# google/lyra

Measured on AMD Instinct MI355X. Metric: 20ms 16kHz frames/sec encode+decode (whole node) at batch 4096; xRT/stream, higher is better.
Workload: dtype f32+i8 (fp32 and int8 layers exactly as the reference graphs)

## Files before the change

lyra_amd/csrc/dec_stages.h:

```cpp
#ifndef LYRA_AMD_CSRC_DEC_STAGES_H_
#define LYRA_AMD_CSRC_DEC_STAGES_H_
#include "resblock_q.h"

namespace lyra {

namespace {
constexpr int SD0 = 8;
constexpr int FS = 72;
constexpr int CS2 = 264;
constexpr int QS = 288;
constexpr int QS5 = 544;
constexpr int NTD0 = 512;
constexpr int MTD0 = (2 * SD0) / 16;
constexpr int FB_FLOATS = 3 * 16 * FS;
constexpr int XF_FLOATS = 2 * SD0 * CS2;
constexpr int H8_BYTES = 16 * QS5;
constexpr int QB_BYTES = 2 * SD0 * QS;
constexpr int QA_BYTES = 2 * 16 * QS;
constexpr int NLR = 6, NADD = 2;
static_assert(SD0 == 8, "tile size the index math below supports");
}

__host__ __device__ constexpr size_t dec_s0_lds() {
  return (size_t)(FB_FLOATS + XF_FLOATS) * 4 + H8_BYTES + 3 * QB_BYTES + QA_BYTES + 2 * SD0 * 4 + NLR * 256 +
// ... 358 lines not shown
      }
    }
  }
}

__host__ __device__ constexpr size_t dec_s1_lds() { return (size_t)(4 * SD1 * CS1 + 4 * SD1 * CS1 + 4 * SD1 * CS1 + 5 * SD1 * 72) * 4 + 2 * SD1 * 4; }

__device__ __forceinline__ void dec_s1_body(const DecS1P& P, const float* __restrict__ in0,
                                            const int32_t* __restrict__ ids, int B, uint8_t* __restrict__ state,
                                            float* __restrict__ out1, int code_bytes, int tile = (int)blockIdx.x) {
  extern __shared__ __attribute__((aligned(16))) float smem[];
  float* XB = smem;
  float* DB = XB + 4 * SD1 * CS1;
  float* PB = DB + 4 * SD1 * CS1;
  float* SB = PB + 4 * SD1 * CS1;
  int* sids = reinterpret_cast<int*>(SB + 5 * SD1 * 72);
  int* sphase = sids + SD1;
  const int tid = threadIdx.x, wave = tid >> 6;
  const int b0 = tile * SD1;
  LYRA_TSTAMP(50);
  int my_id = 0;
  if (tid < SD1) my_id = ids[min(b0 + tid, B - 1)];
  constexpr int XIN = (4 * SD1 * 32) / NTD1;
  static_assert((4 * SD1 * 32) % NTD1 == 0 && (4 * SD1 * 32) / NTD1 >= 1, "the unrolled input prefetch covers the stage input only when the thread count divides it");
  f32x4 xin[XIN];
#pragma unroll
  for (int k = 0; k < XIN; ++k) {
    const int idx = tid + k * NTD1;
    int p4 = idx & 31, s = (idx >> 5) & (SD1 - 1), t = (idx >> 5) / SD1;
    int sb = min(s, B - 1 - b0);
    xin[k] = *goff<const f32x4>(in0 + (size_t)b0 * 512, (uint32_t)(((sb * 4 + t) * 128 + p4 * 4) * 4));
  }
  if (tid < SD1) {
    sids[tid] = my_id;
    sphase[tid] = *reinterpret_cast<const int*>(state + (size_t)max(my_id, 0) * st::D1_BYTES + st::PHASE);
  }
  const auto warm = l2_warm<NTD1, 2>(P.warm);
  const auto warm_code = code_warm<NTD1>(code_bytes);
#pragma unroll
  for (int k = 0; k < XIN; ++k) {
    const int idx = tid + k * NTD1;
    int p4 = idx & 31, s = (idx >> 5) & (SD1 - 1), t = (idx >> 5) / SD1;
    *reinterpret_cast<f32x4*>(&XB[(t * SD1 + s) * CS1 + p4 * 4]) = xin[k];
  }
  LYRA_SYNC_KEEP();
  TileCtx cx{state, sids, sphase, B - b0, st::D1_BYTES};
  const auto H0 = hist128_prefetch<SD1, NTD1>(cx, 1, st::D_R1_0);
  for (int idx = tid; idx < 5 * SD1 * 16; idx += NTD1) {
    int p4 = idx & 15, s = (idx >> 4) & (SD1 - 1), j = (idx >> 4) / SD1;
    *reinterpret_cast<f32x4*>(&SB[(j * SD1 + s) * 72 + p4 * 4]) =
        *cx.at<const f32x4>(cx.soff(s) + (uint32_t)(st::D_UP2 + (j * 64 + p4 * 4) * 4));
  }
  __syncthreads();
  LYRA_TSTAMP(51);
  LYRA_WSTAMP(111);
  resblocks128<SD1, NTD1>(XB, DB, PB, cx, P.dw, P.pw, P.cv, st::D_R1_0, st::D_R1_1, st::D_R1_2, H0);
  LYRA_TSTAMP(52);
  LYRA_WSTAMP(112);
  for (int idx = tid; idx < 4 * SD1 * 32; idx += NTD1) {
    int p4 = idx & 31, rs = idx >> 5;
    f32x4* x = reinterpret_cast<f32x4*>(&XB[rs * CS1 + p4 * 4]);
    *x = lrelu4(*x);
  }
  __syncthreads();
  LYRA_TSTAMP(53);
  LYRA_WSTAMP(113);
  constexpr int HEAD_TILES = NTD1 == 256 ? 5 : 3;
  static_assert((NTD1 / 64) * HEAD_TILES * 256 <= 2 * 4 * SD1 * CS1, "head scratch fits into DB + PB");
  float* HB = DB + wave * (HEAD_TILES * 4 * 64);
  if (NTD1 == 256) dec_s1_tconv<5>(XB, SB, P, cx, b0, out1, wave * 5, HB);
  else if (wave < 4) dec_s1_tconv<3>(XB, SB, P, cx, b0, out1, wave * 3, HB);
  else dec_s1_tconv<2>(XB, SB, P, cx, b0, out1, 12 + (wave - 4) * 2, HB);
  if (tid < SD1 && cx.valid(tid)) {
    int ph = sphase[tid] + 1;
    *cx.at<int>(cx.soff(tid) + (uint32_t)(st::PHASE)) = ph >= st::PHASE_MOD ? 0 : ph;
  }
  l2_warm_sink(warm, state, B);
  l2_warm_sink(warm_code, state, B);
}

namespace {
constexpr int CS0 = 72;
}
__host__ __device__ constexpr size_t dec_s2_lds(int sd2) { return (size_t)(27 * sd2 * CS0 + sd2 * 48) * 4 + 64; }

template <int SD2>
__device__ __forceinline__ void dec_s2_body(const DecS2P& P, const float* __restrict__ in1,
                                            const int32_t* __restrict__ ids, int B, uint8_t* __restrict__ state,
                                            int16_t* __restrict__ pcm, int code_bytes, int tile = (int)blockIdx.x) {
  constexpr int NTD2 = 64 * SD2;
  extern __shared__ __attribute__((aligned(16))) float smem[];
  float* XB = smem;
  float* SB = XB + 27 * SD2 * CS0;
  int* sids = reinterpret_cast<int*>(SB + SD2 * 48);
  const int tid = threadIdx.x, lane = tid & 63, wave = tid >> 6;
  const int m = lane & 15, q = lane >> 4;
  const int b0 = tile * SD2;
  LYRA_TSTAMP(60);
  int my_id = 0;
  if (tid < SD2) my_id = ids[min(b0 + tid, B - 1)];
  const int wn = wave & 3, wm = wave >> 2;
  [[maybe_unused]] const int ncol = wn * 16 + (lane & 15);
  f32x4 xr[5][1];
#pragma unroll
  for (int i = 0; i < 5; ++i) {
    const int R = (wm * 5 + i) * 16 + m, t = R / SD2, s = R & (SD2 - 1);
    const int sb = min(s, B - 1 - b0);
    xr[i][0] = *goff<const f32x4>(in1 + (size_t)b0 * 1280, (uint32_t)(((sb * 20 + t) * 64 + wn * 16 + q * 4) * 4));
  }
  if (tid < SD2) sids[tid] = my_id;
  const auto warm = l2_warm<NTD2, 1>(P.warm);
  const auto warm_code = code_warm<NTD2>(code_bytes);
  LYRA_SYNC_KEEP();
  TileCtx cx{state, sids, nullptr, B - b0, st::D2_BYTES};
  for (int idx = tid; idx < 7 * SD2 * 16; idx += NTD2) {
    int p4 = idx & 15, s = (idx >> 4) & (SD2 - 1), j = (idx >> 4) / SD2;
    int row = j < 3 ? j : 20 + j;
    *reinterpret_cast<f32x4*>(&XB[(row * SD2 + s) * CS0 + p4 * 4]) = (f32x4){0.f, 0.f, 0.f, 0.f};
  }
  for (int idx = tid; idx < SD2 * 48; idx += NTD2) {
    int s = idx / 48, i = idx - s * 48;
    SB[idx] = *cx.at<const float>(cx.soff(s) + (uint32_t)(st::D_UP3 + i * 4));
  }
  LYRA_TSTAMP(61);
  resblocks64r<SD2, NTD2>(xr, XB + 3 * SD2 * CS0, cx, P.dw, P.pw, P.cv, st::D_R2_0, st::D_R2_1, st::D_R2_2);
  LYRA_TSTAMP(62);
#pragma unroll
  for (int i = 0; i < 5; ++i)
{
    const f32x4 a4 = lrelu4(xr[i][0]);
    *reinterpret_cast<f32x4*>(&XB[(3 * SD2 + (wm * 5 + i) * 16 + m) * CS0 + wn * 16 + q * 4]) = a4;
  }
  __syncthreads();
  if (wave < 3 * SD2 / 4) {
    f32x4 acc[2][1];
    auto aoff = [&](int i, int c) {
      int R = (2 * wave + i) * 16 + m, b = R / SD2, s = R & (SD2 - 1);
      return ((b + 3 - (c >> 2)) * SD2 + s) * CS0 + (c & 3) * 16 + q * 4;
    };
    const float bias = as_global(P.up.b)[0];
    const f32x4 bias4[1] = {(f32x4){bias, bias, bias, bias}};
    gemm_f32_init<2, 1, 16, 16, gemm_pf<2, 1>(), true>(XB, aoff, P.up.w, bias4, acc);
#pragma unroll
    for (int i = 0; i < 2; ++i) {
      const int R = (2 * wave + i) * 16 + m, b = R / SD2, s = R & (SD2 - 1);
      if (b > 22) continue;
      const int tau0 = 16 * b + 4 * q;
      f32x4 y = acc[i][0];
      f32x4 old = (f32x4){0.f, 0.f, 0.f, 0.f};
      if (tau0 < 48) old = *reinterpret_cast<const f32x4*>(&SB[s * 48 + tau0]);
#pragma unroll
      for (int e = 0; e < 4; ++e) y[e] = y[e] + old[e];
      if (!cx.valid(s)) continue;
      if (tau0 < 320) {
        int v[4];
#pragma unroll
        for (int e = 0; e < 4; ++e) {
          float f = y[e] * 32768.f;
          f = f < -32768.f ? -32768.f : f;
          f = f > 32767.f ? 32767.f : f;
          v[e] = (int)(int16_t)f;
        }
        typedef int i32x2 __attribute__((ext_vector_type(2)));
        const i32x2 pk = (i32x2){(v[0] & 0xffff) | (v[1] << 16), (v[2] & 0xffff) | (v[3] << 16)};
        *goff<i32x2>(pcm + (size_t)b0 * 320, (uint32_t)((s * 320 + tau0) * 2)) = pk;
      } else {
        f32x4 t;
#pragma unroll
        for (int e = 0; e < 4; ++e) t[e] = y[e] - P.up_sub;
        *cx.at<f32x4>(cx.soff(s) + (uint32_t)(st::D_UP3 + (tau0 - 320) * 4)) = t;
      }
    }
  }
  l2_warm_sink(warm, state, B);
  l2_warm_sink(warm_code, state, B);
}

}
#endif
```

lyra_amd/csrc/enc_stages.h:

```cpp
#ifndef LYRA_AMD_CSRC_ENC_STAGES_H_
#define LYRA_AMD_CSRC_ENC_STAGES_H_
#include "resblocks.h"

namespace lyra {

namespace {
constexpr int CS0 = 72;
constexpr int PBS = 376;
constexpr int S1 = 8;
constexpr int CS1 = 136;
constexpr int NT1 = S1_THREADS;
constexpr int NW1 = NT1 / 64;
}

__host__ __device__ constexpr size_t enc_s0_lds(int s0) { return (size_t)(25 * s0 * CS0) * 4 + 64; }
__host__ __device__ constexpr size_t enc_s1_lds() { return (size_t)(6 * S1 * CS1 + 4 * S1 * CS1 + 4 * S1 * CS1) * 4 + 2 * S1 * 4; }

template <int S0>
__device__ __forceinline__ void enc_s0_body(const EncS0P& P, const int16_t* __restrict__ pcm,
                                            const int32_t* __restrict__ ids, int B, uint8_t* __restrict__ state,
                                            float* __restrict__ out0, int code_bytes, int tile = (int)blockIdx.x) {
  constexpr int NT0 = 64 * S0, NW0 = NT0 / 64;
  extern __shared__ __attribute__((aligned(16))) float smem[];
  float* XB = smem;
  int* sids = reinterpret_cast<int*>(XB + 25 * S0 * CS0);
  static_assert(S0 * PBS <= 25 * S0 * CS0, "PCM staging fits");
  const int tid = threadIdx.x, lane = tid & 63, wave = tid >> 6;
  const int m = lane & 15, q = lane >> 4;
  const int b0 = tile * S0;
  LYRA_WG_BEGIN();
  LYRA_TSTAMP(0);
  LYRA_WSTAMP(100);
  if (tid < S0) sids[tid] = ids[min(b0 + tid, B - 1)];
  const auto warm = l2_warm<NT0, 1>(P.warm);
  const auto warm_code = code_warm<NT0>(code_bytes);
  LYRA_SYNC_KEEP();
  auto soff = [&](int s) -> uint32_t { return (uint32_t)max(sids[s], 0) * (uint32_t)st::E0_BYTES; };
  auto gat = [&](uint32_t o) -> uint8_t LYRA_GLOBAL* { return (uint8_t LYRA_GLOBAL*)state + o; };
  auto valid = [&](int s) -> bool { return b0 + s < B && sids[s] >= 0; };

  f32x4 halo[2];
#pragma unroll
  for (int k = 0; k < 2; ++k) {
    const int idx = tid + k * NT0;
    const int p4 = idx & 15, s = (idx >> 4) & (S0 - 1), j = (idx >> 4) / S0;
    halo[k] = (f32x4){0.f, 0.f, 0.f, 0.f};
    if (idx < 5 * S0 * 16) halo[k] = *(const f32x4 LYRA_GLOBAL*)gat(soff(s) + (uint32_t)(st::E_D0 + (j * 64 + p4 * 4) * 4));
  }

  float* PB = XB;
  for (int idx = tid; idx < S0 * 46; idx += NT0) {
    int s = idx / 46, v = idx - s * 46;
    float x[8];
    if (v < 6) {
      const f32x4 LYRA_GLOBAL* h = (const f32x4 LYRA_GLOBAL*)gat(soff(s) + (uint32_t)(st::E_FIRST + v * 32));
      f32x4 a = h[0], b = h[1];
      x[0] = a[0]; x[1] = a[1]; x[2] = a[2]; x[3] = a[3]; x[4] = b[0]; x[5] = b[1]; x[6] = b[2]; x[7] = b[3];
    } else {
      int sb = min(s, B - 1 - b0);
      i32x4 w = *goff<const i32x4>(pcm + (size_t)b0 * 320, (uint32_t)(sb * 640 + (v - 6) * 16));
#pragma unroll
      for (int e = 0; e < 4; ++e) {
        x[2 * e] = (float)(int16_t)(w[e] & 0xffff) * (1.0f / 32768.0f);
        x[2 * e + 1] = (float)(int16_t)(w[e] >> 16) * (1.0f / 32768.0f);
      }
    }
#pragma unroll
    for (int e = 0; e < 8; ++e) PB[s * PBS + at16(v * 8 + e)] = x[e];
  }
  __syncthreads();
  for (int idx = tid; idx < S0 * 48; idx += NT0) {
    int s = idx / 48, i = idx - s * 48;
    if (valid(s)) *(float LYRA_GLOBAL*)gat(soff(s) + (uint32_t)(st::E_FIRST + i * 4)) = PB[s * PBS + at16(320 + i)];
  }
  LYRA_TSTAMP(1);

  const int wn = wave & 3, wm = wave >> 2;

  f32x4 xr[5][1];
  {
    auto aoff = [&](int i, int c) {
      int R = (wm * 5 + i) * 16 + m;
      return (R & (S0 - 1)) * PBS + (R / S0 + c) * 16 + q * 4;
    };
    gemm_f32_bias<5, 1, 4, 4, gemm_pf<5, 1>(), true>(PB, aoff, P.first.w + wn * 4 * 64, P.first.b, wn * 16, xr);
  }
  __syncthreads();
#pragma unroll
  for (int k = 0; k < 2; ++k) {
    const int idx = tid + k * NT0;
    const int p4 = idx & 15, s = (idx >> 4) & (S0 - 1), j = (idx >> 4) / S0;
    if (idx < 5 * S0 * 16) *reinterpret_cast<f32x4*>(&XB[(j * S0 + s) * CS0 + p4 * 4]) = halo[k];
  }
  LYRA_TSTAMP(2);

  TileCtx cx{state, sids, nullptr, B - b0, st::E0_BYTES};
  resblocks64r<S0, NT0>(xr, XB + 5 * S0 * CS0, cx, P.dw, P.pw, P.cv, st::E_R0_0, st::E_R0_1, st::E_R0_2);
  LYRA_TSTAMP(3);

#pragma unroll
  for (int i = 0; i < 5; ++i)
{
    const f32x4 a4 = lrelu4(xr[i][0]);
    *reinterpret_cast<f32x4*>(&XB[(5 * S0 + (wm * 5 + i) * 16 + m) * CS0 + wn * 16 + q * 4]) = a4;
  }
  __syncthreads();
  for (int idx = tid; idx < 5 * S0 * 16; idx += NT0) {
    int p4 = idx & 15, s = (idx >> 4) & (S0 - 1), j = (idx >> 4) / S0;
    if (valid(s))
      *(f32x4 LYRA_GLOBAL*)gat(soff(s) + (uint32_t)(st::E_D0 + (j * 64 + p4 * 4) * 4)) =
          *reinterpret_cast<const f32x4*>(&XB[((20 + j) * S0 + s) * CS0 + p4 * 4]);
  }
  LYRA_TSTAMP(4);

  {
    constexpr int MTW = (4 * S0) / 16, NTW = 8 / NW0;
    f32x4 acc[MTW][NTW];
    auto aoff = [&](int i, int c) {
      int tap = c >> 2, c16 = c & 3;
      int R = i * 16 + m;
      return ((5 * (R / S0) + tap) * S0 + (R & (S0 - 1))) * CS0 + c16 * 16 + q * 4;
    };
    gemm_f32_bias<MTW, NTW, 40, 40, gemm_pf<MTW, NTW>(), true>(XB, aoff, P.down.w + (wave * NTW) * 40 * 64, P.down.b,
                                                               wave * NTW * 16, acc);
    LYRA_TSTAMP(5);
#pragma unroll
    for (int j = 0; j < NTW; ++j) {
#pragma unroll
      for (int i = 0; i < MTW; ++i) {
        const int R = i * 16 + m, tau = R / S0, s = R & (S0 - 1);
        if (valid(s))
          *goff<f32x4>(out0 + (size_t)b0 * 512, (uint32_t)(((s * 4 + tau) * 128 + (wave * NTW + j) * 16 + q * 4) * 4)) = acc[i][j];
      }
    }
  }
  LYRA_WG_END();
  LYRA_TSTAMP(6);
  LYRA_WSTAMP(101);
  l2_warm_sink(warm, state, B);
  l2_warm_sink(warm_code, state, B);
}

__device__ __forceinline__ void enc_s1_body(const EncS1P& P, const float* __restrict__ in0,
                                            const int32_t* __restrict__ ids, int B, uint8_t* __restrict__ state,
                                            float* __restrict__ out1, int code_bytes, int tile = (int)blockIdx.x) {
  extern __shared__ __attribute__((aligned(16))) float smem[];
  float* XB = smem;
  float* DB = XB + 6 * S1 * CS1;
  float* PB = DB + 4 * S1 * CS1;
  int* sids = reinterpret_cast<int*>(PB + 4 * S1 * CS1);
  int* sphase = sids + S1;
  const int tid = threadIdx.x, lane = tid & 63, wave = tid >> 6;
  const int m = lane & 15, q = lane >> 4;
  const int b0 = tile * S1;
  LYRA_TSTAMP(70);
  LYRA_WSTAMP(102);
  int my_id = 0;
  if (tid < S1) my_id = ids[min(b0 + tid, B - 1)];
  constexpr int XIN = (4 * S1 * 32) / NT1;
  static_assert((4 * S1 * 32) % NT1 == 0 && (4 * S1 * 32) / NT1 >= 1, "the unrolled input prefetch covers the stage input only when the thread count divides it");
  f32x4 xin[XIN];
#pragma unroll
  for (int k = 0; k < XIN; ++k) {
    const int idx = tid + k * NT1;
    int p4 = idx & 31, s = (idx >> 5) & (S1 - 1), t = (idx >> 5) / S1;
    int sb = min(s, B - 1 - b0);
    xin[k] = *goff<const f32x4>(in0 + (size_t)b0 * 512, (uint32_t)(((sb * 4 + t) * 128 + p4 * 4) * 4));
  }
  if (tid < S1) {
    sids[tid] = my_id;
    sphase[tid] = *reinterpret_cast<const int*>(state + (size_t)max(my_id, 0) * st::E1_BYTES + st::PHASE);
  }
  const auto warm = l2_warm<NT1, 2>(P.warm);
  const auto warm_code = code_warm<NT1>(code_bytes);
#pragma unroll
  for (int k = 0; k < XIN; ++k) {
    const int idx = tid + k * NT1;
    int p4 = idx & 31, s = (idx >> 5) & (S1 - 1), t = (idx >> 5) / S1;
    *reinterpret_cast<f32x4*>(&XB[((2 + t) * S1 + s) * CS1 + p4 * 4]) = xin[k];
  }
// ... 66 lines not shown
```

lyra_amd/csrc/lyra_dev.h:

```cpp
#pragma once
#include <hip/hip_runtime.h>
#include <stdint.h>

#define LYRA_SYNC_KEEP() do { __builtin_amdgcn_fence(__ATOMIC_RELEASE, "workgroup"); __builtin_amdgcn_s_barrier(); \
                              __builtin_amdgcn_fence(__ATOMIC_ACQUIRE, "workgroup"); } while (0)

typedef float f32x4 __attribute__((ext_vector_type(4)));
typedef int i32x4 __attribute__((ext_vector_type(4)));

#define LYRA_LRELU_ALPHA 0.30000001192092896f

#ifdef LYRA_TIMING
static __device__ long long g_lyra_tdbg[128];
static __device__ int g_lyra_exit_at = -1;
#define LYRA_TSTAMP(i) do { if (blockIdx.x == 0 && threadIdx.x == 0) g_lyra_tdbg[i] = clock64(); \
    if (g_lyra_exit_at == (i)) return; } while (0)
#define LYRA_WSTAMP(i) do { if (blockIdx.x == 0 && threadIdx.x == 0) g_lyra_tdbg[i] = wall_clock64(); } while (0)
#define LYRA_TSTAMP2(i) do { if (blockIdx.x == 0 && threadIdx.x == 0) g_lyra_tdbg[i] = clock64(); } while (0)
static __device__ long long g_lyra_wgtrace[2048 * 4];
#define LYRA_WG_BEGIN() do { if (threadIdx.x == 0 && blockIdx.x < 2048) { \
    g_lyra_wgtrace[blockIdx.x * 4 + 0] = wall_clock64(); \
    g_lyra_wgtrace[blockIdx.x * 4 + 2] = __builtin_amdgcn_s_getreg(63492); \
    g_lyra_wgtrace[blockIdx.x * 4 + 3] = __builtin_amdgcn_s_getreg(63508); } } while (0)
#define LYRA_WG_END() do { if (threadIdx.x == 0 && blockIdx.x < 2048) g_lyra_wgtrace[blockIdx.x * 4 + 1] = wall_clock64(); } while (0)
#else
#define LYRA_WG_BEGIN() do { } while (0)
#define LYRA_WG_END() do { } while (0)
#define LYRA_WSTAMP(i) do { } while (0)
#define LYRA_TSTAMP(i) do { } while (0)
#define LYRA_TSTAMP2(i) do { } while (0)
#endif

#ifdef LYRA_STRESS_DELAY
#define LYRA_STRESS(bit) do { if (((LYRA_STRESS_DELAY) >> (bit)) & 1) for (int i_ = 0; i_ < 60; ++i_) __builtin_amdgcn_s_sleep(127); } while (0)
#else
#define LYRA_STRESS(bit) do { } while (0)
#endif

namespace lyra {

__host__ __device__ constexpr int at16(int k) { return (k & ~15) | ((k & 3) << 2) | ((k >> 2) & 3); }

__device__ __forceinline__ float lrelu(float x) {
  const float ax = x * LYRA_LRELU_ALPHA;
  float r;
  asm("v_max_f32 %0, %1, %2" : "=v"(r) : "v"(x), "v"(ax));
  return r;
}
typedef float f32x2 __attribute__((ext_vector_type(2)));
__device__ __forceinline__ f32x4 lrelu4(f32x4 v) {
  f32x4 r;
  const f32x2 al = (f32x2){LYRA_LRELU_ALPHA, LYRA_LRELU_ALPHA};
  f32x2 lo = (f32x2){v[0], v[1]}, hi = (f32x2){v[2], v[3]}, alo, ahi;
  alo = lo * al;
  ahi = hi * al;
  asm("v_max_f32 %0, %1, %2" : "=v"(r[0]) : "v"(v[0]), "v"(alo[0]));
  asm("v_max_f32 %0, %1, %2" : "=v"(r[1]) : "v"(v[1]), "v"(alo[1]));
  asm("v_max_f32 %0, %1, %2" : "=v"(r[2]) : "v"(v[2]), "v"(ahi[0]));
  asm("v_max_f32 %0, %1, %2" : "=v"(r[3]) : "v"(v[3]), "v"(ahi[1]));
  return r;
}
__device__ __forceinline__ f32x4 fma4(f32x4 a, f32x4 b, f32x4 c) {
  f32x4 r;
  r[0] = __builtin_fmaf(a[0], b[0], c[0]); r[1] = __builtin_fmaf(a[1], b[1], c[1]);
  r[2] = __builtin_fmaf(a[2], b[2], c[2]); r[3] = __builtin_fmaf(a[3], b[3], c[3]);
  return r;
}

__device__ __forceinline__ int32_t srdhm(int32_t a, int32_t b) {
  const int64_t p = (int64_t)a * (int64_t)b + (1ll << 30);
  return (int32_t)(p >> 31);
}
__device__ __forceinline__ int32_t rdivpot(int32_t x, int e) {
  const int32_t mask = (int32_t)((1u << e) - 1u);
  const int32_t rem = x & mask;
  const int32_t thr = (mask >> 1) + (x < 0 ? 1 : 0);
  return (x >> e) + (rem > thr ? 1 : 0);
}
__device__ __forceinline__ int32_t mbqm_double(int32_t x, int32_t M, int shift) {
  const int left = shift > 0 ? shift : 0;
  const int right = shift > 0 ? 0 : -shift;
  return rdivpot(srdhm((int32_t)((uint32_t)x << left), M), right);
}
__device__ __forceinline__ int32_t mbqm_exact(int32_t x, int32_t M, int shift) {
  int total = 31 - shift;
// ... 35 lines not shown
  const float lo = (float)(-128 - z), hi = (float)(127 - z);
  const float c = __builtin_amdgcn_fmed3f(v, lo, hi);
  return __float_as_int(c + 12582912.f) - (0x4B400000 - z);
}
__device__ __forceinline__ int32_t xnn_requant(int32_t acc, int32_t Mbits, int32_t zout) {
  return rne_clamped_code((float)acc * __int_as_float(Mbits), zout);
}
template <int MODE, bool UNGROUPED_CONV>
__host__ __device__ constexpr int conv_flavour() { return MODE == 3 ? (UNGROUPED_CONV ? 0 : 1) : MODE; }
template <int MODE>
__device__ __forceinline__ int32_t conv_code(int32_t acc, int32_t M, int sh, int32_t zout) {
  static_assert(MODE >= 0 && MODE <= 2, "a layer's flavour (conv_flavour<>), not the kernel's mode");
  if constexpr (MODE == 2) return xnn_requant(acc, M, zout);
  else return clamp8(requant(acc, M, sh, MODE) + zout);
}
template <int MODE>
__device__ __forceinline__ float conv_dequant(int32_t acc, int32_t M, int sh, int32_t zout, float s_dq) {
  if constexpr (MODE == 2) {
    const float lo = (float)(-128 - zout), hi = (float)(127 - zout);
    const float c = __builtin_amdgcn_fmed3f((float)acc * __int_as_float(M), lo, hi);
    const float r = (c + 12582912.f) - 12582912.f;
    return s_dq * r;
  } else {
    return dequantize_f(conv_code<MODE>(acc, M, sh, zout), s_dq, zout);
  }
}
__device__ __forceinline__ int32_t xnn_quantize(float x, const QP& Q) { return rne_clamped_code(x * Q.rs, Q.z); }
template <int MODE>
__device__ __forceinline__ int32_t quantize_code(float x, const QP& Q) {
  if constexpr (MODE == 2) return xnn_quantize(x, Q);
  else return quantize_f(x, Q);
}
__device__ __forceinline__ int32_t xnn_add(int32_t a, int32_t b, const AddQ& L) {
  const int32_t acc = L.mo + a * L.m1 + b * L.m2;
  return clamp8((acc >> L.so) + L.zo);
}

#define LYRA_GLOBAL __attribute__((address_space(1)))
template <class T>
__device__ __forceinline__ const T LYRA_GLOBAL* as_global(const T* p) {
  return (const T LYRA_GLOBAL*)p;
}
template <class T, class U>
__device__ __forceinline__ T LYRA_GLOBAL* goff(U* base, uint32_t byte_off) {
  return (T LYRA_GLOBAL*)((uint8_t LYRA_GLOBAL*)base + byte_off);
}
template <class T>
__device__ __forceinline__ const T LYRA_GLOBAL* wave_uniform(const T* p) {
  const uint64_t v = (uint64_t)p;
  const uint32_t lo = __builtin_amdgcn_readfirstlane((uint32_t)v), hi = __builtin_amdgcn_readfirstlane((uint32_t)(v >> 32));
  return (const T LYRA_GLOBAL*)(((uint64_t)hi << 32) | lo);
}

template <int NTW, int PF>
struct WPre { f32x4 b[PF][NTW]; f32x4 init[NTW]; };

__device__ __forceinline__ f32x4 bias_quad(const float* bias, int n0) {
  return *reinterpret_cast<const f32x4 LYRA_GLOBAL*>(as_global(bias) + n0 + (((threadIdx.x & 63) >> 4) << 2));
}

template <int NTW, int KC, int KS, int PF, bool SWAP = false>
__device__ __forceinline__ WPre<NTW, PF> gemm_f32_wprefetch(const f32x4* bfrag_generic, const float* bias, int n0) {
  const int lane = threadIdx.x & 63;
  const f32x4 LYRA_GLOBAL* bbase = wave_uniform(bfrag_generic);
  WPre<NTW, PF> pre;
#pragma unroll
  for (int p = 0; p < PF; ++p)
#pragma unroll
    for (int j = 0; j < NTW; ++j) pre.b[p][j] = bbase[(j * KS + (p < KC ? p : 0)) * 64 + lane];
  if constexpr (SWAP) {
#pragma unroll
    for (int j = 0; j < NTW; ++j) pre.init[j] = bias_quad(bias, n0 + j * 16);
  } else {
    const float LYRA_GLOBAL* b = as_global(bias) + n0 + (threadIdx.x & 15);
#pragma unroll
    for (int j = 0; j < NTW; ++j) {
      const float v = b[j * 16];
      pre.init[j] = (f32x4){v, v, v, v};
    }
  }
  return pre;
}

template <int MTW, int NTW, int KC, int KS, int INIT, int PF, bool SWAP = false, class AOff>
__device__ __forceinline__ void gemm_f32_core(const float* lds, AOff a_off, const f32x4* bfrag_generic,
                                              f32x4 (&acc)[MTW][NTW], const f32x4 (&init)[NTW],
                                              const f32x4 (*pre_b)[NTW] = nullptr) {
  const int lane = threadIdx.x & 63;
  const f32x4 LYRA_GLOBAL* bbase = wave_uniform(bfrag_generic);
  if (INIT == 2) {
#pragma unroll
    for (int j = 0; j < NTW; ++j) acc[MTW - 1][j] = init[j];
  }
  f32x4 bq[PF + 1][NTW], aq[PF + 1][MTW];
#pragma unroll
  for (int p = 0; p < PF; ++p)
    if (p < KC) {
#pragma unroll
      for (int j = 0; j < NTW; ++j) bq[p][j] = pre_b ? pre_b[p][j] : bbase[(j * KS + p) * 64 + lane];
#pragma unroll
      for (int i = 0; i < MTW; ++i) aq[p][i] = *reinterpret_cast<const f32x4*>(lds + a_off(i, p));
    }
#pragma unroll
  for (int c = 0; c < KC; ++c) {
    if (c + PF < KC) {
      const int sl = (c + PF) % (PF + 1);
#pragma unroll
      for (int j = 0; j < NTW; ++j) bq[sl][j] = bbase[(j * KS + (c + PF)) * 64 + lane];
#pragma unroll
      for (int i = 0; i < MTW; ++i) aq[sl][i] = *reinterpret_cast<const f32x4*>(lds + a_off(i, c + PF));
    }
    const int cur = c % (PF + 1);
#pragma unroll
    for (int kk = 0; kk < 4; ++kk)
#pragma unroll
      for (int i = 0; i < MTW; ++i)
#pragma unroll
        for (int j = 0; j < NTW; ++j) {
          const bool first = c == 0 && kk == 0;
          const f32x4 cin = (first && INIT == 0) ? (f32x4){0.f, 0.f, 0.f, 0.f} : (first && INIT == 2) ? acc[MTW - 1][j] : acc[i][j];
          acc[i][j] = SWAP ? __builtin_amdgcn_mfma_f32_16x16x4f32(bq[cur][j][kk], aq[cur][i][kk], cin, 0, 0, 0)
                           : __builtin_amdgcn_mfma_f32_16x16x4f32(aq[cur][i][kk], bq[cur][j][kk], cin, 0, 0, 0);
        }
  }
}

template <int MTW, int NTW, int KC, int KS = KC, bool ZERO = true,
          int PF = (4 * MTW * NTW >= 16 ? 1 : (4 * MTW * NTW >= 8 ? 2 : 3)), class AOff>
__device__ __forceinline__ void gemm_f32(const float* lds, AOff a_off, const f32x4* bfrag_generic,
                                         f32x4 (&acc)[MTW][NTW]) {
  f32x4 none[NTW];
  gemm_f32_core<MTW, NTW, KC, KS, ZERO ? 0 : 1, PF>(lds, a_off, bfrag_generic, acc, none);
}

template <int MTW, int NTW, int KC, int KS = KC,
          int PF = (4 * MTW * NTW >= 16 ? 1 : (4 * MTW * NTW >= 8 ? 2 : 3)), bool SWAP = false, class AOff>
__device__ __forceinline__ void gemm_f32_bias(const float* lds, AOff a_off, const f32x4* bfrag_generic,
                                              const float* bias, int n0, f32x4 (&acc)[MTW][NTW]) {
  f32x4 init[NTW];
  if constexpr (SWAP) {
#pragma unroll
    for (int j = 0; j < NTW; ++j) init[j] = bias_quad(bias, n0 + j * 16);
  } else {
    const float LYRA_GLOBAL* b = as_global(bias) + n0 + (threadIdx.x & 15);
#pragma unroll
    for (int j = 0; j < NTW; ++j) {
      const float v = b[j * 16];
      init[j] = (f32x4){v, v, v, v};
    }
  }
  gemm_f32_core<MTW, NTW, KC, KS, 2, PF, SWAP>(lds, a_off, bfrag_generic, acc, init);
}

template <int MTW, int NTW, int KC, int KS = KC,
          int PF = (4 * MTW * NTW >= 16 ? 1 : (4 * MTW * NTW >= 8 ? 2 : 3)), bool SWAP = false, class AOff>
__device__ __forceinline__ void gemm_f32_pre(const float* lds, AOff a_off, const f32x4* bfrag_generic,
                                             const WPre<NTW, PF>& pre, f32x4 (&acc)[MTW][NTW]) {
  gemm_f32_core<MTW, NTW, KC, KS, 2, PF, SWAP>(lds, a_off, bfrag_generic, acc, pre.init, pre.b);
}
template <int MTW, int NTW>
constexpr int gemm_pf() { return 4 * MTW * NTW >= 16 ? 1 : (4 * MTW * NTW >= 8 ? 2 : 3); }

template <int MTW, int NTW, int KC, int KS = KC,
          int PF = (4 * MTW * NTW >= 16 ? 1 : (4 * MTW * NTW >= 8 ? 2 : 3)), bool SWAP = false, class AOff>
__device__ __forceinline__ void gemm_f32_init(const float* lds, AOff a_off, const f32x4* bfrag_generic,
                                              const f32x4 (&init)[NTW], f32x4 (&acc)[MTW][NTW]) {
  gemm_f32_core<MTW, NTW, KC, KS, 2, PF, SWAP>(lds, a_off, bfrag_generic, acc, init);
}

template <int MTW, int NTW, int KC, class AOff>
__device__ __forceinline__ void gemm_i8(const int8_t* lds, AOff a_off, const i32x4* bfrag_generic,
                                        i32x4 (&acc)[MTW][NTW]) {
  const int lane = threadIdx.x & 63;
  const i32x4 LYRA_GLOBAL* bfrag = wave_uniform(bfrag_generic);
#pragma unroll
  for (int i = 0; i < MTW; ++i)
#pragma unroll
    for (int j = 0; j < NTW; ++j) acc[i][j] = (i32x4){0, 0, 0, 0};
#pragma unroll
  for (int c = 0; c < KC; ++c) {
    i32x4 b[NTW], a[MTW];
#pragma unroll
    for (int j = 0; j < NTW; ++j) b[j] = bfrag[(j * KC + c) * 64 + lane];
#pragma unroll
    for (int i = 0; i < MTW; ++i) a[i] = *reinterpret_cast<const i32x4*>(lds + a_off(i, c));
#pragma unroll
    for (int i = 0; i < MTW; ++i)
#pragma unroll
      for (int j = 0; j < NTW; ++j)
        acc[i][j] = __builtin_amdgcn_mfma_i32_16x16x64_i8(a[i], b[j], acc[i][j], 0, 0, 0);
  }
}

template <int NTW, int KC, class AOff>
__device__ __forceinline__ void gemm_i8_t(const int8_t* lds, AOff a_off, const i32x4* bfrag_generic, i32x4 (&acc)[NTW]) {
  const int lane = threadIdx.x & 63;
  const i32x4 LYRA_GLOBAL* bfrag = wave_uniform(bfrag_generic);
#pragma unroll
  for (int c = 0; c < KC; ++c) {
    i32x4 w[NTW];
#pragma unroll
    for (int j = 0; j < NTW; ++j) w[j] = bfrag[(j * KC + c) * 64 + lane];
    const i32x4 a = *reinterpret_cast<const i32x4*>(lds + a_off(c));
#pragma unroll
    for (int j = 0; j < NTW; ++j) acc[j] = __builtin_amdgcn_mfma_i32_16x16x64_i8(w[j], a, acc[j], 0, 0, 0);
  }
}
__device__ __forceinline__ i32x4 chan_quad(const int32_t* p, int nt) {
  return *reinterpret_cast<const i32x4 LYRA_GLOBAL*>(as_global(p) + nt * 16 + (((threadIdx.x & 63) >> 4) << 2));
}

template <int H>
__device__ __forceinline__ void fold_rows8(i32x4 (&acc)[2 * H]) {
#pragma unroll
  for (int j = 0; j < H; ++j)
#pragma unroll
    for (int e = 0; e < 4; ++e)
      acc[j][e] = (int)__builtin_amdgcn_permlane32_swap((unsigned)acc[j][e], (unsigned)acc[j + H][e], false, false)[0];
}
template <int H>
__device__ __forceinline__ void fold_rows8(f32x4 (&acc)[2 * H]) {
#pragma unroll
  for (int j = 0; j < H; ++j)
#pragma unroll
    for (int e = 0; e < 4; ++e)
      acc[j][e] = __uint_as_float(__builtin_amdgcn_permlane32_swap(__float_as_uint(acc[j][e]),
                                                                   __float_as_uint(acc[j + H][e]), false, false)[0]);
}

__device__ __forceinline__ void rot32_pair(float& a, float& b) {
  auto r1 = __builtin_amdgcn_permlane32_swap(__float_as_uint(a), __float_as_uint(b), false, false);
  auto r2 = __builtin_amdgcn_permlane32_swap(r1[1], r1[0], false, false);
  a = __uint_as_float(r2[0]);
  b = __uint_as_float(r2[1]);
// ... 48 lines not shown
```

lyra_amd/csrc/resblocks.h:

```cpp
#pragma once
#include "kernels.h"

namespace lyra {

struct TileCtx {
  uint8_t* state;
  const int* sids;
  const int* sphase;
  int nvalid;
  int stride;
  __device__ __forceinline__ uint8_t* sbase(int s) const { return state + (size_t)max(sids[s], 0) * stride; }
  __device__ __forceinline__ bool valid(int s) const { return s < nvalid && sids[s] >= 0; }
  __device__ __forceinline__ uint32_t soff(int s) const { return (uint32_t)max(sids[s], 0) * (uint32_t)stride; }
  template <class T>
  __device__ __forceinline__ T LYRA_GLOBAL* at(uint32_t byte_off) const {
    return (T LYRA_GLOBAL*)((uint8_t LYRA_GLOBAL*)state + byte_off);
  }
};

template <int S, int NT>
__device__ __forceinline__ uint32_t state_touch(const TileCtx& cx, int off, int bytes) {
  const int l0 = off >> 7, n = ((off + bytes - 1) >> 7) - l0 + 1;
  const int idx = threadIdx.x;
  uint32_t tok = 0;
  if (idx < S * n) {
    const int s = idx / n, l = idx - s * n;
    tok = *cx.at<const uint32_t>(cx.soff(s) + (uint32_t)((l0 + l) << 7));
  }
  return tok;
}
__device__ __forceinline__ void state_touch_sink(uint32_t tok, uint8_t* state, int B) {
  if (tok == 0x9E3779B9u && B == -0x5EED) state[0] = (uint8_t)tok;
}

template <int S, int NT>
__device__ __forceinline__ void resblocks64r(f32x4 (&xr)[5][1], float* A, const TileCtx& cx, const DwF* dws,
                                             const ConvF* pws, const ConvF* cvs, int off0, int off1, int off2) {
  constexpr int CS = 72;
  static_assert(20 * S / 16 == 5 * (NT / 256), "5 M tiles per wave");
#pragma unroll 1
  for (int r = 0; r < 3; ++r) {
    int tid = threadIdx.x;
    asm volatile("" : "+v"(tid));
    const int lane = tid & 63, wave = tid >> 6;
    const int m = lane & 15, q = lane >> 4;
    const int wn = wave & 3, wm = wave >> 2;
    [[maybe_unused]] const int ncol = wn * 16 + (lane & 15);
    const int d = r == 0 ? 1 : (r == 1 ? 3 : 9);
    const int R2 = 2 * d;
    const int off = r == 0 ? off0 : (r == 1 ? off1 : off2);
    LYRA_TSTAMP(10 + r * 8 + 0);
    constexpr int RSTEP = NT / 16;
    const int p4 = tid & 15, rq = tid >> 4;
    const float LYRA_GLOBAL* dww = as_global(dws[r].w);
    static_assert(RSTEP % S == 0, "one stream per thread");
    constexpr int TSTEP = RSTEP / S;
    const int sq = rq & (S - 1), tq = rq / S;
    const uint32_t hb0 = cx.soff(sq) + (uint32_t)(off + (tq * 64 + p4 * 4) * 4);
    const uint32_t hb1 = hb0 + (uint32_t)(d * 256);
    f32x4 h0[5], h1[5];
#pragma unroll
    for (int k = 0; k < 5; ++k) {
      const int t = tq + k * TSTEP;
      h0[k] = (f32x4){0.f, 0.f, 0.f, 0.f};
      h1[k] = (f32x4){0.f, 0.f, 0.f, 0.f};
      if (t < 2 * d) h0[k] = *cx.at<const f32x4>(hb0 + k * TSTEP * 256);
      if (t < d) h1[k] = *cx.at<const f32x4>(hb1 + k * TSTEP * 256);
    }
#pragma unroll
    for (int i = 0; i < 5; ++i)
{
      const f32x4 a4 = lrelu4(xr[i][0]);
      *reinterpret_cast<f32x4*>(&A[((wm * 5 + i) * 16 + m) * CS + wn * 16 + q * 4]) = a4;
    }
    __syncthreads();
    LYRA_TSTAMP(10 + r * 8 + 1);
    f32x4 dreg[5];
    {
      const f32x4 w0 = *reinterpret_cast<const f32x4 LYRA_GLOBAL*>(dww + p4 * 4);
#pragma unroll
      for (int k = 0; k < 5; ++k) {
        const int t0 = tq + k * TSTEP - 2 * d;
        const f32x4 v0 = t0 >= 0 ? *reinterpret_cast<const f32x4*>(&A[(t0 * S + sq) * CS + p4 * 4]) : h0[k];
        dreg[k] = fma4(v0, w0, (f32x4){0.f, 0.f, 0.f, 0.f});
      }
      const f32x4 w1 = *reinterpret_cast<const f32x4 LYRA_GLOBAL*>(dww + 64 + p4 * 4);
#pragma unroll
      for (int k = 0; k < 5; ++k) {
        const int t1 = tq + k * TSTEP - d;
        const f32x4 v1 = t1 >= 0 ? *reinterpret_cast<const f32x4*>(&A[(t1 * S + sq) * CS + p4 * 4]) : h1[k];
        dreg[k] = fma4(v1, w1, dreg[k]);
      }
      const f32x4 w2 = *reinterpret_cast<const f32x4 LYRA_GLOBAL*>(dww + 128 + p4 * 4);
#pragma unroll
      for (int k = 0; k < 5; ++k) {
        const f32x4 v2 = *reinterpret_cast<const f32x4*>(&A[(rq + k * RSTEP) * CS + p4 * 4]);
        dreg[k] = fma4(v2, w2, dreg[k]);
      }
    }
    LYRA_TSTAMP(10 + r * 8 + 2);
    __syncthreads();
#pragma unroll
    for (int k = 0; k < 5; ++k) {
      f32x4* item = reinterpret_cast<f32x4*>(&A[(rq + k * RSTEP) * CS + p4 * 4]);
      const int j = tq + k * TSTEP - (20 - R2);
      if (j >= 0 && cx.valid(sq)) *cx.at<f32x4>(cx.soff(sq) + (uint32_t)(off + (j * 64 + p4 * 4) * 4)) = *item;
      *item = dreg[k];
    }
    __syncthreads();
    LYRA_TSTAMP(10 + r * 8 + 4);
    auto aoff = [&](int i, int c) { return ((wm * 5 + i) * 16 + m) * CS + c * 16 + q * 4; };
    WPre<1, 1> cv_pre;
    {
      f32x4 acc[5][1];
      gemm_f32_bias<5, 1, 4, 4, gemm_pf<5, 1>(), true>(A, aoff, pws[r].w + wn * 4 * 64, pws[r].b, wn * 16, acc);
      LYRA_TSTAMP(10 + r * 8 + 5);
      cv_pre = gemm_f32_wprefetch<1, 4, 4, 1, true>(cvs[r].w + wn * 4 * 64, cvs[r].b, wn * 16);
      __syncthreads();
#pragma unroll
      for (int i = 0; i < 5; ++i)
{
        const f32x4 a4 = lrelu4(acc[i][0]);
        *reinterpret_cast<f32x4*>(&A[((wm * 5 + i) * 16 + m) * CS + wn * 16 + q * 4]) = a4;
      }
      __syncthreads();
      LYRA_TSTAMP(10 + r * 8 + 6);
    }
    {
      f32x4 acc[5][1];
      gemm_f32_pre<5, 1, 4, 4, gemm_pf<5, 1>(), true>(A, aoff, cvs[r].w + wn * 4 * 64, cv_pre, acc);
#pragma unroll
      for (int i = 0; i < 5; ++i)
#pragma unroll
        for (int e = 0; e < 4; ++e) xr[i][0][e] = acc[i][0][e] + xr[i][0][e];
    }
    LYRA_TSTAMP(10 + r * 8 + 7);
    __syncthreads();
  }
}

template <int RPT>
struct Hist128 { f32x4 h[RPT][2]; };

template <int S, int NT>
__device__ __forceinline__ Hist128<1024 / NT> hist128_prefetch(const TileCtx& cx, int d, int off) {
  constexpr int RPT = 1024 / NT;
  const int tid = threadIdx.x, p4 = tid & 31, s = (tid >> 5) & (S - 1), row0 = (tid >> 8) * RPT;
  const int R2 = 2 * d;
  const bool ring = R2 > 4;
  const int base = ring ? (cx.sphase[s] * 4) % R2 : 0;
  const uint32_t hp = cx.soff(s) + (uint32_t)(off + p4 * 16);
  Hist128<RPT> H;
#pragma unroll
  for (int k = 0; k < RPT; ++k)
#pragma unroll
    for (int j = 0; j < 2; ++j) {
      const int tau = row0 + k - (2 - j) * d;
      H.h[k][j] = (f32x4){0.f, 0.f, 0.f, 0.f};
      if (tau < 0) {
        int row = R2 + tau;
        if (ring) { row = base + tau + R2; row = row >= R2 ? row - R2 : row; }
        H.h[k][j] = *cx.at<const f32x4>(hp + (uint32_t)(row * 512));
      }
    }
  return H;
}

template <int S, int NT>
__device__ __forceinline__ void resblocks128(float* X, float* D, float* P, const TileCtx& cx, const DwF* dws,
                                             const ConvF* pws, const ConvF* cvs, int off0, int off1, int off2,
                                             Hist128<1024 / NT> H) {
  static_assert(S == 8 && (NT == 256 || NT == 512), "thread <-> (stream, channel quad, row half) mapping");
  constexpr int CS = 136, NTW = 8 / (NT / 64), MT = 2, RPT = 1024 / NT;
  constexpr int PF = gemm_pf<MT, NTW>();
#pragma unroll 1
  for (int r = 0; r < 3; ++r) {
    int tid = threadIdx.x;
    asm volatile("" : "+v"(tid));
    const int lane = tid & 63, wave = tid >> 6;
    const int m = lane & 15, q = lane >> 4;
    const int p4 = tid & 31, s = (tid >> 5) & (S - 1), row0 = (tid >> 8) * RPT;
    const int d = r == 0 ? 1 : (r == 1 ? 3 : 9);
    const int R2 = 2 * d;
    const int off = r == 0 ? off0 : (r == 1 ? off1 : off2);
    const bool ring = R2 > 4;
    LYRA_TSTAMP(40 + r * 8 + 0);
    {
      const float LYRA_GLOBAL* dww = as_global(dws[r].w) + p4 * 4;
      const f32x4 w0 = *reinterpret_cast<const f32x4 LYRA_GLOBAL*>(dww);
      const f32x4 w1 = *reinterpret_cast<const f32x4 LYRA_GLOBAL*>(dww + 128);
      const f32x4 w2 = *reinterpret_cast<const f32x4 LYRA_GLOBAL*>(dww + 256);
      const uint32_t hp = cx.soff(s) + (uint32_t)(off + p4 * 16);
      const int base = ring ? (cx.sphase[s] * 4) % R2 : 0;
      const bool valid = cx.valid(s);
      const float* xq = &X[s * CS + p4 * 4];
#pragma unroll
      for (int k = 0; k < RPT; ++k) {
        const int t = row0 + k, t0 = t - 2 * d, t1 = t - d;
        const f32x4 a = lrelu4(*reinterpret_cast<const f32x4*>(xq + t * S * CS));
        f32x4 v0 = H.h[k][0], v1 = H.h[k][1];
        if (t0 >= 0) v0 = lrelu4(*reinterpret_cast<const f32x4*>(xq + t0 * S * CS));
        if (t1 >= 0) v1 = lrelu4(*reinterpret_cast<const f32x4*>(xq + t1 * S * CS));
        f32x4 acc = fma4(v0, w0, (f32x4){0.f, 0.f, 0.f, 0.f});
        acc = fma4(v1, w1, acc);
        acc = fma4(a, w2, acc);
        *reinterpret_cast<f32x4*>(&D[(t * S + s) * CS + p4 * 4]) = acc;
        if (valid) {
          if (ring) {
            int row = base + t;
            row = row >= R2 ? row - R2 : row;
            *cx.at<f32x4>(hp + (uint32_t)(row * 512)) = a;
          } else if (t >= 2) {
            *cx.at<f32x4>(hp + (uint32_t)((t - 2) * 512)) = a;
          }
        }
      }
    }
    const auto pw_pre = gemm_f32_wprefetch<NTW, 8, 8, PF>(pws[r].w + (wave * NTW) * 8 * 64, pws[r].b, wave * NTW * 16);
    WPre<NTW, PF> cv_pre;
// ... 49 lines not shown
```

Measured before the change: 14.38 million.

## Stage resblock dilated-conv history rows into LDS via async global_load_lds

For 4-stream tiles, the dilated-conv history rows for the resblocks are copied straight into LDS with global_load_lds_dwordx4. Rows for dilations 1 and 3 are issued at stage start, and rows for dilation 9 are issued from a hook inside the pointwise GEMM's last K step. This replaces per-thread register gathers of history with asynchronous copies that overlap compute. The cost is extra LDS per block (which may lower occupancy), inline asm that sets m0, and vmcnt waits.

```diff
diff --git a/lyra_amd/csrc/dec_stages.h b/lyra_amd/csrc/dec_stages.h
--- a/lyra_amd/csrc/dec_stages.h
+++ b/lyra_amd/csrc/dec_stages.h
@@ -464,7 +464,7 @@
 namespace {
 constexpr int CS0 = 72;
 }
-__host__ __device__ constexpr size_t dec_s2_lds(int sd2) { return (size_t)(27 * sd2 * CS0 + sd2 * 48) * 4 + 64; }
+__host__ __device__ constexpr size_t dec_s2_lds(int sd2) { return (size_t)(27 * sd2 * CS0 + sd2 * 48) * 4 + 64 + hist64_lds(sd2); }
 
 template <int SD2>
 __device__ __forceinline__ void dec_s2_body(const DecS2P& P, const float* __restrict__ in1,
@@ -475,6 +475,7 @@
   float* XB = smem;
   float* SB = XB + 27 * SD2 * CS0;
   int* sids = reinterpret_cast<int*>(SB + SD2 * 48);
+  float* H = reinterpret_cast<float*>(sids) + 16;
   const int tid = threadIdx.x, lane = tid & 63, wave = tid >> 6;
   const int m = lane & 15, q = lane >> 4;
   const int b0 = tile * SD2;
@@ -495,6 +496,10 @@
   const auto warm_code = code_warm<NTD2>(code_bytes);
   LYRA_SYNC_KEEP();
   TileCtx cx{state, sids, nullptr, B - b0, st::D2_BYTES};
+  if constexpr (hist64_lds(SD2) != 0) {
+    static_assert(st::D_R2_1 == st::D_R2_0 + 2 * 256 && st::D_R2_2 == st::D_R2_1 + 6 * 256 && HIST64_ROWS == 8, "rows 0-7 from D_R2_0");
+    hist64_to_lds<SD2, NTD2>(cx, H, st::D_R2_0);
+  }
   for (int idx = tid; idx < 7 * SD2 * 16; idx += NTD2) {
     int p4 = idx & 15, s = (idx >> 4) & (SD2 - 1), j = (idx >> 4) / SD2;
     int row = j < 3 ? j : 20 + j;
@@ -505,7 +510,7 @@
     SB[idx] = *cx.at<const float>(cx.soff(s) + (uint32_t)(st::D_UP3 + i * 4));
   }
   LYRA_TSTAMP(61);
-  resblocks64r<SD2, NTD2>(xr, XB + 3 * SD2 * CS0, cx, P.dw, P.pw, P.cv, st::D_R2_0, st::D_R2_1, st::D_R2_2);
+  resblocks64r<SD2, NTD2>(xr, XB + 3 * SD2 * CS0, H, cx, P.dw, P.pw, P.cv, st::D_R2_0, st::D_R2_1, st::D_R2_2);
   LYRA_TSTAMP(62);
 #pragma unroll
   for (int i = 0; i < 5; ++i)
diff --git a/lyra_amd/csrc/enc_stages.h b/lyra_amd/csrc/enc_stages.h
--- a/lyra_amd/csrc/enc_stages.h
+++ b/lyra_amd/csrc/enc_stages.h
@@ -13,7 +13,7 @@
 constexpr int NW1 = NT1 / 64;
 }
 
-__host__ __device__ constexpr size_t enc_s0_lds(int s0) { return (size_t)(25 * s0 * CS0) * 4 + 64; }
+__host__ __device__ constexpr size_t enc_s0_lds(int s0) { return (size_t)(25 * s0 * CS0) * 4 + 64 + hist64_lds(s0); }
 __host__ __device__ constexpr size_t enc_s1_lds() { return (size_t)(6 * S1 * CS1 + 4 * S1 * CS1 + 4 * S1 * CS1) * 4 + 2 * S1 * 4; }
 
 template <int S0>
@@ -24,6 +24,7 @@
   extern __shared__ __attribute__((aligned(16))) float smem[];
   float* XB = smem;
   int* sids = reinterpret_cast<int*>(XB + 25 * S0 * CS0);
+  float* H = reinterpret_cast<float*>(sids) + 16;
   static_assert(S0 * PBS <= 25 * S0 * CS0, "PCM staging fits");
   const int tid = threadIdx.x, lane = tid & 63, wave = tid >> 6;
   const int m = lane & 15, q = lane >> 4;
@@ -47,6 +48,10 @@
     halo[k] = (f32x4){0.f, 0.f, 0.f, 0.f};
     if (idx < 5 * S0 * 16) halo[k] = *(const f32x4 LYRA_GLOBAL*)gat(soff(s) + (uint32_t)(st::E_D0 + (j * 64 + p4 * 4) * 4));
   }
+  if constexpr (hist64_lds(S0) != 0) {
+    static_assert(st::E_R0_1 == st::E_R0_0 + 2 * 256 && st::E_R0_2 == st::E_R0_1 + 6 * 256 && HIST64_ROWS == 8, "rows 0-7 from E_R0_0");
+    hist64_to_lds<S0, NT0>(TileCtx{state, sids, nullptr, B - b0, st::E0_BYTES}, H, st::E_R0_0);
+  }
 
   float* PB = XB;
   for (int idx = tid; idx < S0 * 46; idx += NT0) {
@@ -95,7 +100,7 @@
   LYRA_TSTAMP(2);
 
   TileCtx cx{state, sids, nullptr, B - b0, st::E0_BYTES};
-  resblocks64r<S0, NT0>(xr, XB + 5 * S0 * CS0, cx, P.dw, P.pw, P.cv, st::E_R0_0, st::E_R0_1, st::E_R0_2);
+  resblocks64r<S0, NT0>(xr, XB + 5 * S0 * CS0, H, cx, P.dw, P.pw, P.cv, st::E_R0_0, st::E_R0_1, st::E_R0_2);
   LYRA_TSTAMP(3);
 
 #pragma unroll
diff --git a/lyra_amd/csrc/lyra_dev.h b/lyra_amd/csrc/lyra_dev.h
--- a/lyra_amd/csrc/lyra_dev.h
+++ b/lyra_amd/csrc/lyra_dev.h
@@ -1,6 +1,7 @@
 #pragma once
 #include <hip/hip_runtime.h>
 #include <stdint.h>
+#include <type_traits>
 
 #define LYRA_SYNC_KEEP() do { __builtin_amdgcn_fence(__ATOMIC_RELEASE, "workgroup"); __builtin_amdgcn_s_barrier(); \
                               __builtin_amdgcn_fence(__ATOMIC_ACQUIRE, "workgroup"); } while (0)
@@ -202,10 +203,12 @@
   return pre;
 }
 
-template <int MTW, int NTW, int KC, int KS, int INIT, int PF, bool SWAP = false, class AOff>
+struct GemmNoHook { __device__ __forceinline__ void operator()(float) const {} };
+
+template <int MTW, int NTW, int KC, int KS, int INIT, int PF, bool SWAP = false, class AOff, class LastK = GemmNoHook>
 __device__ __forceinline__ void gemm_f32_core(const float* lds, AOff a_off, const f32x4* bfrag_generic,
                                               f32x4 (&acc)[MTW][NTW], const f32x4 (&init)[NTW],
-                                              const f32x4 (*pre_b)[NTW] = nullptr) {
+                                              const f32x4 (*pre_b)[NTW] = nullptr, LastK lastk = LastK()) {
   const int lane = threadIdx.x & 63;
   const f32x4 LYRA_GLOBAL* bbase = wave_uniform(bfrag_generic);
   if (INIT == 2) {
@@ -231,6 +234,9 @@
       for (int i = 0; i < MTW; ++i) aq[sl][i] = *reinterpret_cast<const f32x4*>(lds + a_off(i, c + PF));
     }
     const int cur = c % (PF + 1);
+    if constexpr (!std::is_same<LastK, GemmNoHook>::value) {
+      if (c == KC - 1) lastk(bq[cur][0][0]);
+    }
 #pragma unroll
     for (int kk = 0; kk < 4; ++kk)
 #pragma unroll
@@ -254,9 +260,10 @@
 }
 
 template <int MTW, int NTW, int KC, int KS = KC,
-          int PF = (4 * MTW * NTW >= 16 ? 1 : (4 * MTW * NTW >= 8 ? 2 : 3)), bool SWAP = false, class AOff>
+          int PF = (4 * MTW * NTW >= 16 ? 1 : (4 * MTW * NTW >= 8 ? 2 : 3)), bool SWAP = false, class AOff,
+          class LastK = GemmNoHook>
 __device__ __forceinline__ void gemm_f32_bias(const float* lds, AOff a_off, const f32x4* bfrag_generic,
-                                              const float* bias, int n0, f32x4 (&acc)[MTW][NTW]) {
+                                              const float* bias, int n0, f32x4 (&acc)[MTW][NTW], LastK lastk = LastK()) {
   f32x4 init[NTW];
   if constexpr (SWAP) {
 #pragma unroll
@@ -269,7 +276,7 @@
       init[j] = (f32x4){v, v, v, v};
     }
   }
-  gemm_f32_core<MTW, NTW, KC, KS, 2, PF, SWAP>(lds, a_off, bfrag_generic, acc, init);
+  gemm_f32_core<MTW, NTW, KC, KS, 2, PF, SWAP>(lds, a_off, bfrag_generic, acc, init, nullptr, lastk);
 }
 
 template <int MTW, int NTW, int KC, int KS = KC,
diff --git a/lyra_amd/csrc/resblocks.h b/lyra_amd/csrc/resblocks.h
--- a/lyra_amd/csrc/resblocks.h
+++ b/lyra_amd/csrc/resblocks.h
@@ -33,11 +33,38 @@
   if (tok == 0x9E3779B9u && B == -0x5EED) state[0] = (uint8_t)tok;
 }
 
-template <int S, int NT>
-__device__ __forceinline__ void resblocks64r(f32x4 (&xr)[5][1], float* A, const TileCtx& cx, const DwF* dws,
+constexpr int HIST64_ROWS = 8;
+__host__ __device__ constexpr size_t hist64_lds(int s) { return s == 4 ? (size_t)HIST64_ROWS * 4 * 64 * 4 : 0; }
+
+__device__ __forceinline__ void glds16(const uint8_t* state, uint32_t voff, uint32_t lds_base, float dep = 0.f) {
+  uint32_t keep;
+  asm volatile("s_mov_b32 %0, m0\n\ts_mov_b32 m0, %3\n\ts_nop 0\n\tglobal_load_lds_dwordx4 %1, %2\n\ts_mov_b32 m0, %0"
+               : "=&s"(keep)
+               : "v"(voff), "s"((const uint8_t LYRA_GLOBAL*)state), "s"(lds_base), "v"(dep)
+               : "memory");
+}
+
+template <int S, int NT>
+__device__ __forceinline__ void hist64_to_lds(const TileCtx& cx, float* H, int off, float dep = 0.f) {
+  static_assert(S == 4 && NT == 256, "one wave instruction = one row of four streams");
+  const int lane = threadIdx.x & 63, wave = __builtin_amdgcn_readfirstlane(threadIdx.x >> 6);
+  const uint32_t h0 = (uint32_t)(uintptr_t)(__attribute__((address_space(3))) float*)H;
+  const uint32_t src = cx.soff(lane >> 4) + (uint32_t)(off + (lane & 15) * 16);
+#pragma unroll
+  for (int j = 0; j < HIST64_ROWS / 4; ++j) {
+    const int row = wave + 4 * j;
+    glds16(cx.state, src + (uint32_t)(row * 256), __builtin_amdgcn_readfirstlane(h0 + (uint32_t)(row * S * 256)), dep);
+  }
+}
+__device__ __forceinline__ void hist64_retire() { asm volatile("s_waitcnt vmcnt(0)" ::: "memory"); }
+
+template <int S, int NT>
+__device__ __forceinline__ void resblocks64r(f32x4 (&xr)[5][1], float* A, float* H, const TileCtx& cx, const DwF* dws,
                                              const ConvF* pws, const ConvF* cvs, int off0, int off1, int off2) {
   constexpr int CS = 72;
+  constexpr bool HL = hist64_lds(S) != 0;
   static_assert(20 * S / 16 == 5 * (NT / 256), "5 M tiles per wave");
+  if constexpr (HL) hist64_retire();
 #pragma unroll 1
   for (int r = 0; r < 3; ++r) {
     int tid = threadIdx.x;
@@ -49,6 +76,7 @@
     const int d = r == 0 ? 1 : (r == 1 ? 3 : 9);
     const int R2 = 2 * d;
     const int off = r == 0 ? off0 : (r == 1 ? off1 : off2);
+    [[maybe_unused]] const int hrow = r == 1 ? 2 : 0;
     LYRA_TSTAMP(10 + r * 8 + 0);
     constexpr int RSTEP = NT / 16;
     const int p4 = tid & 15, rq = tid >> 4;
@@ -58,14 +86,17 @@
     const int sq = rq & (S - 1), tq = rq / S;
     const uint32_t hb0 = cx.soff(sq) + (uint32_t)(off + (tq * 64 + p4 * 4) * 4);
     const uint32_t hb1 = hb0 + (uint32_t)(d * 256);
+    constexpr int HK = HL ? HIST64_ROWS / TSTEP : 0;
+    static_assert(!HL || HK * TSTEP == HIST64_ROWS, "H ends on an item boundary");
+    const bool hreg = !HL || r == 2;
     f32x4 h0[5], h1[5];
 #pragma unroll
     for (int k = 0; k < 5; ++k) {
       const int t = tq + k * TSTEP;
       h0[k] = (f32x4){0.f, 0.f, 0.f, 0.f};
       h1[k] = (f32x4){0.f, 0.f, 0.f, 0.f};
-      if (t < 2 * d) h0[k] = *cx.at<const f32x4>(hb0 + k * TSTEP * 256);
-      if (t < d) h1[k] = *cx.at<const f32x4>(hb1 + k * TSTEP * 256);
+      if (k >= HK && hreg && t < 2 * d) h0[k] = *cx.at<const f32x4>(hb0 + k * TSTEP * 256);
+      if (hreg && t < d) h1[k] = *cx.at<const f32x4>(hb1 + k * TSTEP * 256);
     }
 #pragma unroll
     for (int i = 0; i < 5; ++i)
@@ -81,14 +112,28 @@
 #pragma unroll
       for (int k = 0; k < 5; ++k) {
         const int t0 = tq + k * TSTEP - 2 * d;
-        const f32x4 v0 = t0 >= 0 ? *reinterpret_cast<const f32x4*>(&A[(t0 * S + sq) * CS + p4 * 4]) : h0[k];
+        f32x4 v0;
+        if constexpr (HL) {
+          v0 = h0[k];
+          if (t0 >= 0) v0 = *reinterpret_cast<const f32x4*>(&A[(t0 * S + sq) * CS + p4 * 4]);
+          else if (r < 2 || k < HK) v0 = *reinterpret_cast<const f32x4*>(&H[((hrow + tq + k * TSTEP) * S + sq) * 64 + p4 * 4]);
+        } else {
+          v0 = t0 >= 0 ? *reinterpret_cast<const f32x4*>(&A[(t0 * S + sq) * CS + p4 * 4]) : h0[k];
+        }
         dreg[k] = fma4(v0, w0, (f32x4){0.f, 0.f, 0.f, 0.f});
       }
       const f32x4 w1 = *reinterpret_cast<const f32x4 LYRA_GLOBAL*>(dww + 64 + p4 * 4);
 #pragma unroll
       for (int k = 0; k < 5; ++k) {
         const int t1 = tq + k * TSTEP - d;
-        const f32x4 v1 = t1 >= 0 ? *reinterpret_cast<const f32x4*>(&A[(t1 * S + sq) * CS + p4 * 4]) : h1[k];
+        f32x4 v1;
+        if constexpr (HL) {
+          v1 = h1[k];
+          if (t1 >= 0) v1 = *reinterpret_cast<const f32x4*>(&A[(t1 * S + sq) * CS + p4 * 4]);
+          else if (r < 2) v1 = *reinterpret_cast<const f32x4*>(&H[((hrow + d + tq + k * TSTEP) * S + sq) * 64 + p4 * 4]);
+        } else {
+          v1 = t1 >= 0 ? *reinterpret_cast<const f32x4*>(&A[(t1 * S + sq) * CS + p4 * 4]) : h1[k];
+        }
         dreg[k] = fma4(v1, w1, dreg[k]);
       }
       const f32x4 w2 = *reinterpret_cast<const f32x4 LYRA_GLOBAL*>(dww + 128 + p4 * 4);
@@ -113,7 +158,15 @@
     WPre<1, 1> cv_pre;
     {
       f32x4 acc[5][1];
-      gemm_f32_bias<5, 1, 4, 4, gemm_pf<5, 1>(), true>(A, aoff, pws[r].w + wn * 4 * 64, pws[r].b, wn * 16, acc);
+      if constexpr (HL) {
+        auto hist9 = [&](float dep) {
+          asm volatile("" : : "v"(dep));
+          if (r == 1) hist64_to_lds<S, NT>(cx, H, off2);
+        };
+        gemm_f32_bias<5, 1, 4, 4, gemm_pf<5, 1>(), true>(A, aoff, pws[r].w + wn * 4 * 64, pws[r].b, wn * 16, acc, hist9);
+      } else {
+        gemm_f32_bias<5, 1, 4, 4, gemm_pf<5, 1>(), true>(A, aoff, pws[r].w + wn * 4 * 64, pws[r].b, wn * 16, acc);
+      }
       LYRA_TSTAMP(10 + r * 8 + 5);
       cv_pre = gemm_f32_wprefetch<1, 4, 4, 1, true>(cvs[r].w + wn * 4 * 64, cvs[r].b, wn * 16);
       __syncthreads();
@@ -135,6 +188,7 @@
         for (int e = 0; e < 4; ++e) xr[i][0][e] = acc[i][0][e] + xr[i][0][e];
     }
     LYRA_TSTAMP(10 + r * 8 + 7);
+    if constexpr (HL) hist64_retire();
     __syncthreads();
   }
 }
```

After: 13.86 million. 3.6% lower.
